# CHONSPQX/modulated-deform-conv

Hardware: AMD Instinct MI355X
Metric: fwd+bwd GSamples/s, MDCN2d 3x3 C=256 56x56 B=32; %HBM roofline (higher is better)
Workload: dtype f32; 1 GPU; ModulatedDeformConv2d 3x3, C_in=C_out=256, 56x56, deformable_group=1, fp32, B=32 per GPU, forward+backward (BASELINE.json configs[1]); global_batch=32, parallelism=dp1 batch-sharded

## Files before the change

### modulated_deform_conv_amd/csrc/mfma_fwd.hip

```cpp
#include "mfma_kernels.hpp"

#include <stdio.h>
#include <stdlib.h>
#include <string.h>

#include "mfma_tile.hpp"

namespace mdconv {

namespace {


template <int ND, bool MOD, int BM, int BN, int WM, int WN, bool PADK>
__global__ __launch_bounds__(256) void mfma_fwd_kernel(Geom g, PackDims pd,
                                                       const float *__restrict__ input,
                                                       const float *__restrict__ wp,
                                                       const float *__restrict__ bias,
                                                       const float *__restrict__ offset,
                                                       const float *__restrict__ mask,
                                                       float *__restrict__ output, int ntm, int ntn,
                                                       int full_tiles, int tail_ways, int tail_hi,
                                                       float *__restrict__ part) {
  constexpr int BK = kBK;
  constexpr int NC = 1 << ND;
  constexpr int NP = NC / 2;
  constexpr int MB = WM / 32, NB = WN / 32;
  constexpr int WAVES_N = BN / WN;
  constexpr int KSUBS = 256 / BN;
  constexpr int CPT = BK / KSUBS;
  static_assert((BM / WM) * (BN / WN) == 4, "4 waves per workgroup");
  static_assert(BK == 16 && CPT >= 1 && BN <= 256 && MB * 2 * 1024 <= 4096, "tile shape");

  __shared__ __attribute__((aligned(16))) float Bs[2 * BK * BN];

  const int grp = blockIdx.y;
  int tile, tap_lo = 0, tap_hi = g.K, tail_slot = -1;
  if ((int)blockIdx.x < full_tiles) {
    tile = xcd_remap(blockIdx.x, full_tiles);
  } else {
    tail_slot = blockIdx.x - full_tiles;
    const int hi_slots = tail_hi * (tail_ways + 1);
    int ti, way, wt;
    if (tail_slot < hi_slots) {
      wt = tail_ways + 1;
      ti = tail_slot / wt;
      way = tail_slot - ti * wt;
    } else {
      wt = tail_ways;
      const int r = tail_slot - hi_slots;
      ti = tail_hi + r / wt;
      way = r - (r / wt) * wt;
    }
    tile = full_tiles + ti;
    tap_lo = way * g.K / wt;
    tap_hi = (way + 1) * g.K / wt;
  }
  const int tn = tile / ntm, tm = tile - tn * ntm;
  const int o0 = tm * BM;
  const int n0 = tn * BN;

  const int tid = threadIdx.x;
  const int lane = tid & 63;
  const int wave = __builtin_amdgcn_readfirstlane(tid >> 6);
  const int wm0 = (wave / WAVES_N) * WM, wn0 = (wave % WAVES_N) * WN;
  const int kh = lane >> 5;

  const int j = tid % BN, ksub = tid / BN;
  const int n_g = min(n0 + j, g.N - 1);
  const int b_g = n_g / g.S_o;
  const int pix_g = n_g - b_g * g.S_o;
  int oc[ND];
  out_coords<ND>(g, pix_g, oc);

  const int cchunks = pd.Cgp / BK;
  const int T = g.K * cchunks;
  const int mblks = pd.Ogp / 32;
  const int slab_bytes = mblks * 2 * 64 * 4 * 4;

  const rsrc_t r_in = make_rsrc(input, (size_t)g.B * g.C * g.S_i * sizeof(float));
  const rsrc_t r_wp = make_rsrc(wp + (size_t)grp * T * (slab_bytes / 4), (size_t)T * slab_bytes);
  const int a_voff = (((o0 + wm0) / 32) * 2 * 64 + lane) * 16;
  const int img_voff = (b_g * g.C + grp * g.Cg + ksub * CPT) * g.S_i * 4;

  f32x16 acc[MB][NB];
#pragma unroll
  for (int i = 0; i < MB; ++i)
#pragma unroll
    for (int k = 0; k < NB; ++k)
#pragma unroll
      for (int r = 0; r < 16; ++r) acc[i][k][r] = 0.f;

  int voff[NP];
  float wgt[NC];
  float2 rg0[CPT][NP], rg1[CPT][NP];
  float wc0[NC], wc1[NC];
  int cur_tap = -1, cur_dg = -1;
  typedef unsigned long long lanemask_t;
  lanemask_t bad[NC], bad0[NC], bad1[NC];
#pragma unroll
  for (int ci = 0; ci < NC; ++ci) bad[ci] = bad0[ci] = bad1[ci] = 0ull;

  auto issue = [&](float2 (&rg)[CPT][NP], float (&wc)[NC], lanemask_t (&bd)[NC], int tap, int c0) {
    const int dg = g.DG == 1 ? 0 : min(grp * g.Cg + c0, g.C - 1) / g.Cdg;
    if (tap != cur_tap || dg != cur_dg) {
      float delta[ND];
      const int64_t ob = ((int64_t)(b_g * g.DG + dg) * (ND * g.K) + ND * tap) * g.S_o + pix_g;
#pragma unroll
      for (int a = 0; a < ND; ++a) delta[a] = offset[ob + (int64_t)a * g.S_o];
      int tcd[ND];
      tap_coords<ND>(g, tap, tcd);
      TapCoef<ND, float> tc;
      make_tap<ND, float>(g, oc, tcd, delta, false, tc);
      const float m = MOD ? mask[((int64_t)(b_g * g.DG + dg) * g.K + tap) * g.S_o + pix_g] : 1.f;
      int pidx[NP];
      float pwx[NP], pwy[NP];
      make_pairs<ND, float>(g, tc, m, pidx, pwx, pwy);
      bool prx[NP], pry[NP];
      make_pairs_read<ND, float>(g, tc, prx, pry);
#pragma unroll
      for (int pi = 0; pi < NP; ++pi) {
        voff[pi] = (prx[pi] || pry[pi]) ? img_voff + pidx[pi] * 4 : 0x7ffffff0;
        wgt[2 * pi] = pwx[pi];
        wgt[2 * pi + 1] = pwy[pi];
        bad[2 * pi] = __ballot(pry[pi] && !prx[pi]);
        bad[2 * pi + 1] = __ballot(prx[pi] && !pry[pi]);
      }
      cur_tap = tap;
      cur_dg = dg;
    }
    const int soff = c0 * g.S_i * 4;
#pragma unroll
    for (int i = 0; i < CPT; ++i)
#pragma unroll
      for (int pi = 0; pi < NP; ++pi) {
        rg[i][pi] = buf_load2(r_in, voff[pi], soff + i * g.S_i * 4);
      }
#pragma unroll
    for (int ci = 0; ci < NC; ++ci) { wc[ci] = wgt[ci]; bd[ci] = bad[ci]; }
  };
  auto commit = [&](const float2 (&rgl)[CPT][NP], const float (&wc)[NC], const lanemask_t (&bd)[NC], int c0, float *Bb) {
    lanemask_t any_bad = 0ull;
#pragma unroll
    for (int ci = 0; ci < NC; ++ci) any_bad |= bd[ci];
    float2 rg[CPT][NP];
#pragma unroll
    for (int i = 0; i < CPT; ++i)
#pragma unroll
      for (int pi = 0; pi < NP; ++pi) rg[i][pi] = rgl[i][pi];
    if (any_bad != 0ull) {
#pragma unroll
      for (int i = 0; i < CPT; ++i)
#pragma unroll
        for (int pi = 0; pi < NP; ++pi) {
          asm("v_cndmask_b32_e64 %0, %1, 0, %2" : "=v"(rg[i][pi].x) : "v"(rgl[i][pi].x), "s"(bd[2 * pi]));
          asm("v_cndmask_b32_e64 %0, %1, 0, %2" : "=v"(rg[i][pi].y) : "v"(rgl[i][pi].y), "s"(bd[2 * pi + 1]));
        }
    }
#pragma unroll
    for (int i = 0; i < CPT; ++i) {
      float val = wc[0] * rg[i][0].x;
      val = fmaf(wc[1], rg[i][0].y, val);
#pragma unroll
      for (int pi = 1; pi < NP; ++pi) {
        val = fmaf(wc[2 * pi], rg[i][pi].x, val);
        val = fmaf(wc[2 * pi + 1], rg[i][pi].y, val);
      }
      if (PADK) {
        const int cl = c0 + ksub * CPT + i;
        val = cl < g.Cg ? val : 0.f;
      }
      Bb[(ksub * CPT + i) * BN + j] = val;
    }
  };
  auto load_a = [&](float4 (&ra)[MB][2], int soff) {
#pragma unroll
    for (int i = 0; i < MB; ++i)
#pragma unroll
      for (int q = 0; q < 2; ++q) {
        ra[i][q] = buf_load4(r_wp, a_voff + (i * 2 + q) * 1024, soff);
      }
  };
  auto mma = [&](const float4 (&ra)[MB][2], const float *Bbuf) {
    const float *Bb = Bbuf + wn0 + (lane & 31) + 4 * kh * BN;
#pragma unroll
    for (int q = 0; q < 2; ++q)
#pragma unroll
      for (int s = 0; s < 4; ++s) {
        float b[NB];
#pragma unroll
        for (int n = 0; n < NB; ++n) b[n] = Bb[(8 * q + s) * BN + n * 32];
#pragma unroll
        for (int i = 0; i < MB; ++i) {
          const float a = s == 0 ? ra[i][q].x : (s == 1 ? ra[i][q].y : (s == 2 ? ra[i][q].z : ra[i][q].w));
#pragma unroll
          for (int n = 0; n < NB; ++n)
            acc[i][n] = __builtin_amdgcn_mfma_f32_32x32x2f32(a, b[n], acc[i][n], 0, 0, 0);
        }
      }
  };

  float4 ra0[MB][2], ra1[MB][2];
  const int a_last = (T - 1) * slab_bytes;
  int a_soff = tap_lo * cchunks * slab_bytes;
  load_a(ra0, a_soff);
  issue(rg0, wc0, bad0, tap_lo, 0);
  issue(rg1, wc1, bad1, tap_lo, BK);
  for (int tap = tap_lo; tap < tap_hi; ++tap) {
    for (int c0 = 0; c0 < pd.Cgp; c0 += 2 * BK) {
      const bool wrap = c0 + 2 * BK >= pd.Cgp;
      const int ntap = wrap ? min(tap + 1, g.K - 1) : tap;
      const int nc0 = wrap ? 0 : c0 + 2 * BK;
      commit(rg0, wc0, bad0, c0, Bs);
      __syncthreads();
      load_a(ra1, a_soff + slab_bytes);
      issue(rg0, wc0, bad0, ntap, nc0);
      __builtin_amdgcn_sched_barrier(0);
      mma(ra0, Bs);
      commit(rg1, wc1, bad1, c0 + BK, Bs + BK * BN);
      __syncthreads();
      a_soff += 2 * slab_bytes;
      load_a(ra0, min(a_soff, a_last));
      issue(rg1, wc1, bad1, ntap, nc0 + BK);
      __builtin_amdgcn_sched_barrier(0);
      mma(ra1, Bs + BK * BN);
    }
  }

  if (tail_slot >= 0) {
    float *dst = part + (size_t)tail_slot * (BM * BN) + wn0 + (lane & 31);
#pragma unroll
    for (int q = 0; q < NB; ++q)
#pragma unroll
      for (int mb = 0; mb < MB; ++mb)
#pragma unroll
        for (int r = 0; r < 16; ++r)
          dst[(wm0 + mb * 32 + (r & 3) + 8 * (r >> 2) + 4 * kh) * BN + q * 32] = acc[mb][q][r];
    return;
  }
#pragma unroll
  for (int q = 0; q < NB; ++q) {
    const int n_e = n0 + wn0 + q * 32 + (lane & 31);
    if (n_e < g.N) {
      const int b_e = n_e / g.S_o;
      const int pix_e = n_e - b_e * g.S_o;
#pragma unroll
      for (int mb = 0; mb < MB; ++mb)
#pragma unroll
        for (int r = 0; r < 16; ++r) {
          const int ol = o0 + wm0 + mb * 32 + (r & 3) + 8 * (r >> 2) + 4 * kh;
          if (ol < g.Og) {
            const int och = grp * g.Og + ol;
            const float bv = g.with_bias ? bias[och] : 0.f;
            output[(int64_t)(b_e * g.O + och) * g.S_o + pix_e] = acc[mb][q][r] + bv;
          }
        }
    }
  }
}

constexpr int kTailSlices = 16;
template <int BM, int BN>
__global__ __launch_bounds__(256) void fwd_tail_reduce_kernel(Geom g, const float *__restrict__ part,
                                                              const float *__restrict__ bias,
                                                              float *__restrict__ output, int ntm,
                                                              int full_tiles, int tail_ways, int tail_hi) {
  const int tile = full_tiles + blockIdx.x;
  const int tn = tile / ntm, tm = tile - tn * ntm;
  const int ti = blockIdx.x;
  const int slot0 = ti < tail_hi ? ti * (tail_ways + 1) : tail_hi * (tail_ways + 1) + (ti - tail_hi) * tail_ways;
  const int nways = ti < tail_hi ? tail_ways + 1 : tail_ways;
  const float *src = part + (size_t)slot0 * (BM * BN);
  const int e_lo = blockIdx.y * (BM * BN / kTailSlices);
  for (int e = e_lo + threadIdx.x; e < e_lo + BM * BN / kTailSlices; e += 256) {
    const int ol = tm * BM + e / BN, n = tn * BN + e % BN;
    if (ol >= g.Og || n >= g.N) continue;
    float sacc = src[e];
    for (int w = 1; w < nways; ++w) sacc += src[(size_t)w * (BM * BN) + e];
    const int b = n / g.S_o, pix = n - b * g.S_o;
    output[(int64_t)(b * g.O + ol) * g.S_o + pix] = sacc + (g.with_bias ? bias[ol] : 0.f);
  }
}

}

void fwd_tail_plan(const Geom &g, int tiles, int slots, int *full_tiles, int *ways, int *n_hi) {
  static const int tail_env = getenv("MDCONV_FWD_TAIL") ? atoi(getenv("MDCONV_FWD_TAIL")) : 2;
  *full_tiles = tiles;
  *ways = 1;
  *n_hi = 0;
  if (!tail_env || g.G != 1 || g.K < 2 || slots <= 0) return;
  const int rem = tiles % slots;
  if (rem == 0) return;
  int w = slots / rem;
  const int cap = g.K < 4 ? g.K : 4;
  if (tail_env == 1) {
    if (tiles < slots) return;
    if (w > cap) w = cap;
    if (w < 2) return;
    *full_tiles = tiles - rem;
    *ways = w;
    return;
  }
  if (w >= cap) {
    *full_tiles = tiles - rem;
    *ways = cap;
    return;
  }
  const int hi = slots - rem * w;
  if (w == 1) {
    if (hi == 0) return;
    *full_tiles = tiles - hi;
    *ways = 1;
    *n_hi = hi;
    return;
  }
  *full_tiles = tiles - rem;
  *ways = w;
  *n_hi = hi;
}

int fwd_tail_reduce_launch(int BM, int BN, const Geom &g, const float *part, const float *bias, float *output, int ntm,
                           int tail_tiles, int full_tiles, int ways, int n_hi, hipStream_t stream) {
  if (tail_tiles <= 0) return MDCONV_OK;
#define FWD_TAIL_RED(M, N)                                                                                        \
  hipLaunchKernelGGL((fwd_tail_reduce_kernel<M, N>), dim3(tail_tiles, kTailSlices), dim3(256), 0, stream, g, part, bias, \
                     output, ntm, full_tiles, ways, n_hi)
  if (BM == 256 && BN == 32) FWD_TAIL_RED(256, 32);
  else if (BM == 128 && BN == 64) FWD_TAIL_RED(128, 64);
  else if (BM == 64 && BN == 128) FWD_TAIL_RED(64, 128);
  else if (BM == 64 && BN == 64) FWD_TAIL_RED(64, 64);
  else { set_error("fwd_tail_reduce: no instance for a %d x %d tile", BM, BN); return MDCONV_ELAUNCH; }
#undef FWD_TAIL_RED
  return check_launch("fwd_tail_reduce");
}

namespace {
template <int ND, bool MOD, int BM, int BN, int WM, int WN, bool PADK>
int fwd_tile_slots() {
  static int slots = 0;
  if (!slots) {
    int n = 0;
    (void)hipOccupancyMaxActiveBlocksPerMultiprocessor(
        &n, reinterpret_cast<const void *>(&mfma_fwd_kernel<ND, MOD, BM, BN, WM, WN, PADK>), 256, 0);
    (void)hipGetLastError();
    slots = device_cus() * (n > 0 ? (n < kTailMaxPerCu ? n : kTailMaxPerCu) : 3);
  }
  return slots;
}

template <int ND, bool MOD, int BM, int BN, int WM, int WN, bool PADK>
int launch_fwd_tile_k(const Geom &g, const PackDims &pd, const Tensors &t, const float *wp, float *part,
                      hipStream_t stream) {
  const int ntm = (g.Og + BM - 1) / BM;
  const int ntn = (g.N + BN - 1) / BN;
  int full_tiles, ways, n_hi;
  fwd_tail_plan(g, ntm * ntn, part ? fwd_tile_slots<ND, MOD, BM, BN, WM, WN, PADK>() : 0, &full_tiles, &ways, &n_hi);
  const int tail_tiles = ntm * ntn - full_tiles;
  static const bool debug_plan = getenv("MDCONV_DEBUG_PLAN") != nullptr;
  if (debug_plan)
    fprintf(stderr, "[mdconv] forward plan: %d x %d tile, %d tiles, slots %d, full %d, tail %d x %d tap ranges (%d of them x %d)\n", BM, BN,
            ntm * ntn, part ? fwd_tile_slots<ND, MOD, BM, BN, WM, WN, PADK>() : 0, full_tiles, tail_tiles, ways, n_hi, ways + 1);
  dim3 grid(full_tiles + tail_tiles * ways + n_hi, g.G);
  hipLaunchKernelGGL((mfma_fwd_kernel<ND, MOD, BM, BN, WM, WN, PADK>), grid, dim3(256), 0, stream,
                     g, pd, (const float *)t.input, wp, (const float *)t.bias,
                     (const float *)t.offset, (const float *)t.mask, (float *)t.output, ntm, ntn,
                     full_tiles, ways, n_hi, part);
  int rc = check_launch("mfma_fwd");
  if (rc || tail_tiles == 0) return rc;
  return fwd_tail_reduce_launch(BM, BN, g, part, (const float *)t.bias, (float *)t.output, ntm, tail_tiles, full_tiles, ways,
                                n_hi, stream);
}

template <int ND, bool MOD, int BM, int BN, int WM, int WN>
int launch_fwd_tile(const Geom &g, const PackDims &pd, const Tensors &t, const float *wp, float *part,
                    hipStream_t stream) {
  if (g.Cg % (2 * kBK)) return launch_fwd_tile_k<ND, MOD, BM, BN, WM, WN, true>(g, pd, t, wp, part, stream);
  return launch_fwd_tile_k<ND, MOD, BM, BN, WM, WN, false>(g, pd, t, wp, part, stream);
}

template <int ND, bool MOD>
int launch_fwd(const Geom &g, const PackDims &pd, const Tensors &t, const float *wp, float *part,
               hipStream_t stream) {
  if (pd.BM == 256) return launch_fwd_tile<ND, MOD, 256, 32, 64, 32>(g, pd, t, wp, part, stream);
  if (pd.BM == 128) return launch_fwd_tile<ND, MOD, 128, 64, 64, 32>(g, pd, t, wp, part, stream);
  return launch_fwd_tile<ND, MOD, 64, 128, 64, 32>(g, pd, t, wp, part, stream);
}

}


size_t fwd_tail_bytes(const Geom &g) {
  return g.G == 1 && g.K >= 2 ? (size_t)device_cus() * kTailMaxPerCu * 8192 * sizeof(float) : 0;
}

int mfma_forward_f32(const Geom &g, const PackDims &pd, const Tensors &t, const float *wp, float *part,
                     hipStream_t stream) {
  if (g.nd == 2)
    return g.modulated ? launch_fwd<2, true>(g, pd, t, wp, part, stream)
                       : launch_fwd<2, false>(g, pd, t, wp, part, stream);
  return g.modulated ? launch_fwd<3, true>(g, pd, t, wp, part, stream)
                     : launch_fwd<3, false>(g, pd, t, wp, part, stream);
}

}
```

Baseline: 70.78 GSamples/s.

## Precompute per-tap bilinear sampling state into an LDS table in forward kernel

Adds a templated variant of the forward MFMA kernel that, in a prologue, has the threads of a workgroup split the taps between them, computing offsets, mask, bilinear weights, voffsets and boundary flags once per tap and pixel into a dynamic LDS table. The main loop then fetches each tap's state from LDS at the tap boundary instead of recomputing it from global offset and mask loads inside issue. The table is enabled only when deformable_group is 1, it fits in 64 KiB, and occupancy does not drop. The cost is extra LDS use, a prologue barrier, and a restructured tap-wrap loop.

Result: no change. 71.12 GSamples/s (median of 6 runs) (+0.5%).

```diff
diff --git a/modulated_deform_conv_amd/csrc/mfma_fwd.hip b/modulated_deform_conv_amd/csrc/mfma_fwd.hip
--- a/modulated_deform_conv_amd/csrc/mfma_fwd.hip
+++ b/modulated_deform_conv_amd/csrc/mfma_fwd.hip
@@ -1,5 +1,7 @@
 #include "mfma_kernels.hpp"
 
+#include <map>
+#include <mutex>
 #include <stdio.h>
 #include <stdlib.h>
 #include <string.h>
@@ -11,7 +13,9 @@
 namespace {
 
 
-template <int ND, bool MOD, int BM, int BN, int WM, int WN, bool PADK>
+template <int ND> constexpr int fwd_row_dwords() { return ND == 2 ? 8 : 16; }
+
+template <int ND, bool MOD, int BM, int BN, int WM, int WN, bool PADK, bool TBL>
 __global__ __launch_bounds__(256) void mfma_fwd_kernel(Geom g, PackDims pd,
                                                        const float *__restrict__ input,
                                                        const float *__restrict__ wp,
@@ -32,6 +36,8 @@
   static_assert(BK == 16 && CPT >= 1 && BN <= 256 && MB * 2 * 1024 <= 4096, "tile shape");
 
   __shared__ __attribute__((aligned(16))) float Bs[2 * BK * BN];
+  extern __shared__ __attribute__((aligned(16))) int Tb[];
+  constexpr int ROWD = fwd_row_dwords<ND>();
 
   const int grp = blockIdx.y;
   int tile, tap_lo = 0, tap_hi = g.K, tail_slot = -1;
@@ -80,7 +86,9 @@
   const rsrc_t r_in = make_rsrc(input, (size_t)g.B * g.C * g.S_i * sizeof(float));
   const rsrc_t r_wp = make_rsrc(wp + (size_t)grp * T * (slab_bytes / 4), (size_t)T * slab_bytes);
   const int a_voff = (((o0 + wm0) / 32) * 2 * 64 + lane) * 16;
-  const int img_voff = (b_g * g.C + grp * g.Cg + ksub * CPT) * g.S_i * 4;
+  const int img_base = (b_g * g.C + grp * g.Cg) * g.S_i * 4;
+  const int ksub_voff = ksub * CPT * g.S_i * 4;
+  constexpr int kParked = 0x7ffffff0;
 
   f32x16 acc[MB][NB];
 #pragma unroll
@@ -100,33 +108,93 @@
 #pragma unroll
   for (int ci = 0; ci < NC; ++ci) bad[ci] = bad0[ci] = bad1[ci] = 0ull;
 
+  auto make_state = [&](int tap, int dg, int base, int (&vo)[NP], float (&w)[NC], bool (&bx)[NP], bool (&by)[NP]) {
+    float delta[ND];
+    const int64_t ob = ((int64_t)(b_g * g.DG + dg) * (ND * g.K) + ND * tap) * g.S_o + pix_g;
+#pragma unroll
+    for (int a = 0; a < ND; ++a) delta[a] = offset[ob + (int64_t)a * g.S_o];
+    int tcd[ND];
+    tap_coords<ND>(g, tap, tcd);
+    TapCoef<ND, float> tc;
+    make_tap<ND, float>(g, oc, tcd, delta, false, tc);
+    const float m = MOD ? mask[((int64_t)(b_g * g.DG + dg) * g.K + tap) * g.S_o + pix_g] : 1.f;
+    int pidx[NP];
+    float pwx[NP], pwy[NP];
+    make_pairs<ND, float>(g, tc, m, pidx, pwx, pwy);
+    bool prx[NP], pry[NP];
+    make_pairs_read<ND, float>(g, tc, prx, pry);
+#pragma unroll
+    for (int pi = 0; pi < NP; ++pi) {
+      vo[pi] = (prx[pi] || pry[pi]) ? base + pidx[pi] * 4 : kParked;
+      w[2 * pi] = pwx[pi];
+      w[2 * pi + 1] = pwy[pi];
+      bx[pi] = pry[pi] && !prx[pi];
+      by[pi] = prx[pi] && !pry[pi];
+    }
+  };
+  if (TBL) {
+#pragma unroll 1
+    for (int tap = tap_lo + ksub; tap < tap_hi; tap += KSUBS) {
+      int vo[NP];
+      float w[NC];
+      bool bx[NP], by[NP];
+      make_state(tap, 0, img_base, vo, w, bx, by);
+      int row[ROWD];
+      int flags = 0;
+#pragma unroll
+      for (int pi = 0; pi < NP; ++pi) {
+        row[pi] = vo[pi];
+        flags |= (bx[pi] ? 1 << (2 * pi) : 0) | (by[pi] ? 2 << (2 * pi) : 0);
+      }
+#pragma unroll
+      for (int ci = 0; ci < NC; ++ci) row[NP + ci] = __float_as_int(w[ci]);
+      row[NP + NC] = flags;
+#pragma unroll
+      for (int i = NP + NC + 1; i < ROWD; ++i) row[i] = 0;
+      int *dst = Tb + ((tap - tap_lo) * BN + j) * ROWD;
+#pragma unroll
+      for (int i = 0; i < ROWD; i += 4) *reinterpret_cast<int4 *>(dst + i) = make_int4(row[i], row[i + 1], row[i + 2], row[i + 3]);
+    }
+    __syncthreads();
+  }
+
+  auto fetch_state = [&](int tap) {
+    const int *src = Tb + (min(tap, tap_hi - 1) - tap_lo) * (BN * ROWD) + j * ROWD;
+    int row[ROWD];
+#pragma unroll
+    for (int i = 0; i < ROWD; i += 4) {
+      const int4 q = *reinterpret_cast<const int4 *>(src + i);
+      row[i] = q.x; row[i + 1] = q.y; row[i + 2] = q.z; row[i + 3] = q.w;
+    }
+#pragma unroll
+    for (int pi = 0; pi < NP; ++pi)
+      voff[pi] = max(row[pi], (int)((unsigned)row[pi] + (unsigned)ksub_voff));
+#pragma unroll
+    for (int ci = 0; ci < NC; ++ci) wgt[ci] = __int_as_float(row[NP + ci]);
+    const int flags = row[NP + NC];
+    if (__ballot(flags != 0) != 0ull) {
+#pragma unroll
+      for (int ci = 0; ci < NC; ++ci) bad[ci] = __ballot((flags >> ci) & 1);
+    } else {
+#pragma unroll
+      for (int ci = 0; ci < NC; ++ci) bad[ci] = 0ull;
+    }
+  };
+
   auto issue = [&](float2 (&rg)[CPT][NP], float (&wc)[NC], lanemask_t (&bd)[NC], int tap, int c0) {
-    const int dg = g.DG == 1 ? 0 : min(grp * g.Cg + c0, g.C - 1) / g.Cdg;
-    if (tap != cur_tap || dg != cur_dg) {
-      float delta[ND];
-      const int64_t ob = ((int64_t)(b_g * g.DG + dg) * (ND * g.K) + ND * tap) * g.S_o + pix_g;
-#pragma unroll
-      for (int a = 0; a < ND; ++a) delta[a] = offset[ob + (int64_t)a * g.S_o];
-      int tcd[ND];
-      tap_coords<ND>(g, tap, tcd);
-      TapCoef<ND, float> tc;
-      make_tap<ND, float>(g, oc, tcd, delta, false, tc);
-      const float m = MOD ? mask[((int64_t)(b_g * g.DG + dg) * g.K + tap) * g.S_o + pix_g] : 1.f;
-      int pidx[NP];
-      float pwx[NP], pwy[NP];
-      make_pairs<ND, float>(g, tc, m, pidx, pwx, pwy);
-      bool prx[NP], pry[NP];
-      make_pairs_read<ND, float>(g, tc, prx, pry);
-#pragma unroll
-      for (int pi = 0; pi < NP; ++pi) {
-        voff[pi] = (prx[pi] || pry[pi]) ? img_voff + pidx[pi] * 4 : 0x7ffffff0;
-        wgt[2 * pi] = pwx[pi];
-        wgt[2 * pi + 1] = pwy[pi];
-        bad[2 * pi] = __ballot(pry[pi] && !prx[pi]);
-        bad[2 * pi + 1] = __ballot(prx[pi] && !pry[pi]);
-      }
-      cur_tap = tap;
-      cur_dg = dg;
+    if (!TBL) {
+      const int dg = g.DG == 1 ? 0 : min(grp * g.Cg + c0, g.C - 1) / g.Cdg;
+      if (tap != cur_tap || dg != cur_dg) {
+        bool bx[NP], by[NP];
+        make_state(tap, dg, img_base + ksub_voff, voff, wgt, bx, by);
+#pragma unroll
+        for (int pi = 0; pi < NP; ++pi) {
+          bad[2 * pi] = __ballot(bx[pi]);
+          bad[2 * pi + 1] = __ballot(by[pi]);
+        }
+        cur_tap = tap;
+        cur_dg = dg;
+      }
     }
     const int soff = c0 * g.S_i * 4;
 #pragma unroll
@@ -203,26 +271,35 @@
   const int a_last = (T - 1) * slab_bytes;
   int a_soff = tap_lo * cchunks * slab_bytes;
   load_a(ra0, a_soff);
+  if (TBL) fetch_state(tap_lo);
   issue(rg0, wc0, bad0, tap_lo, 0);
   issue(rg1, wc1, bad1, tap_lo, BK);
+  auto chunk_pair = [&](int c0, int ntap, int nc0) {
+    commit(rg0, wc0, bad0, c0, Bs);
+    __syncthreads();
+    load_a(ra1, a_soff + slab_bytes);
+    issue(rg0, wc0, bad0, ntap, nc0);
+    __builtin_amdgcn_sched_barrier(0);
+    mma(ra0, Bs);
+    commit(rg1, wc1, bad1, c0 + BK, Bs + BK * BN);
+    __syncthreads();
+    a_soff += 2 * slab_bytes;
+    load_a(ra0, min(a_soff, a_last));
+    issue(rg1, wc1, bad1, ntap, nc0 + BK);
+    __builtin_amdgcn_sched_barrier(0);
+    mma(ra1, Bs + BK * BN);
+  };
   for (int tap = tap_lo; tap < tap_hi; ++tap) {
-    for (int c0 = 0; c0 < pd.Cgp; c0 += 2 * BK) {
-      const bool wrap = c0 + 2 * BK >= pd.Cgp;
-      const int ntap = wrap ? min(tap + 1, g.K - 1) : tap;
-      const int nc0 = wrap ? 0 : c0 + 2 * BK;
-      commit(rg0, wc0, bad0, c0, Bs);
-      __syncthreads();
-      load_a(ra1, a_soff + slab_bytes);
-      issue(rg0, wc0, bad0, ntap, nc0);
-      __builtin_amdgcn_sched_barrier(0);
-      mma(ra0, Bs);
-      commit(rg1, wc1, bad1, c0 + BK, Bs + BK * BN);
-      __syncthreads();
-      a_soff += 2 * slab_bytes;
-      load_a(ra0, min(a_soff, a_last));
-      issue(rg1, wc1, bad1, ntap, nc0 + BK);
-      __builtin_amdgcn_sched_barrier(0);
-      mma(ra1, Bs + BK * BN);
+    if (TBL) {
+      for (int c0 = 0; c0 + 2 * BK < pd.Cgp; c0 += 2 * BK) chunk_pair(c0, tap, c0 + 2 * BK);
+      const int ntap = min(tap + 1, g.K - 1);
+      fetch_state(ntap);
+      chunk_pair(pd.Cgp - 2 * BK, ntap, 0);
+    } else {
+      for (int c0 = 0; c0 < pd.Cgp; c0 += 2 * BK) {
+        const bool wrap = c0 + 2 * BK >= pd.Cgp;
+        chunk_pair(c0, wrap ? min(tap + 1, g.K - 1) : tap, wrap ? 0 : c0 + 2 * BK);
+      }
     }
   }
 
@@ -335,17 +412,28 @@
 }
 
 namespace {
+template <int ND, bool MOD, int BM, int BN, int WM, int WN, bool PADK, bool TBL>
+int fwd_tile_occupancy(size_t dyn) {
+  static std::mutex mu;
+  static std::map<size_t, int> cache;
+  std::lock_guard<std::mutex> lock(mu);
+  auto it = cache.find(dyn);
+  if (it != cache.end()) return it->second;
+  int n = 0;
+  (void)hipOccupancyMaxActiveBlocksPerMultiprocessor(
+      &n, reinterpret_cast<const void *>(&mfma_fwd_kernel<ND, MOD, BM, BN, WM, WN, PADK, TBL>), 256, dyn);
+  (void)hipGetLastError();
+  cache[dyn] = n;
+  return n;
+}
+
 template <int ND, bool MOD, int BM, int BN, int WM, int WN, bool PADK>
-int fwd_tile_slots() {
-  static int slots = 0;
-  if (!slots) {
-    int n = 0;
-    (void)hipOccupancyMaxActiveBlocksPerMultiprocessor(
-        &n, reinterpret_cast<const void *>(&mfma_fwd_kernel<ND, MOD, BM, BN, WM, WN, PADK>), 256, 0);
-    (void)hipGetLastError();
-    slots = device_cus() * (n > 0 ? (n < kTailMaxPerCu ? n : kTailMaxPerCu) : 3);
-  }
-  return slots;
+size_t fwd_table_bytes(const Geom &g) {
+  if (g.DG != 1) return 0;
+  const size_t bytes = (size_t)g.K * BN * fwd_row_dwords<ND>() * 4;
+  if (bytes + 2 * kBK * BN * 4 > 64 * 1024) return 0;
+  const int plain = fwd_tile_occupancy<ND, MOD, BM, BN, WM, WN, PADK, false>(0);
+  return fwd_tile_occupancy<ND, MOD, BM, BN, WM, WN, PADK, true>(bytes) >= plain && plain > 0 ? bytes : 0;
 }
 
 template <int ND, bool MOD, int BM, int BN, int WM, int WN, bool PADK>
@@ -353,18 +441,31 @@
                       hipStream_t stream) {
   const int ntm = (g.Og + BM - 1) / BM;
   const int ntn = (g.N + BN - 1) / BN;
+  const size_t tbl = fwd_table_bytes<ND, MOD, BM, BN, WM, WN, PADK>(g);
+  int slots = 0;
+  if (part) {
+    const int n = tbl ? fwd_tile_occupancy<ND, MOD, BM, BN, WM, WN, PADK, true>(tbl)
+                      : fwd_tile_occupancy<ND, MOD, BM, BN, WM, WN, PADK, false>(0);
+    slots = device_cus() * (n > 0 ? (n < kTailMaxPerCu ? n : kTailMaxPerCu) : 3);
+  }
   int full_tiles, ways, n_hi;
-  fwd_tail_plan(g, ntm * ntn, part ? fwd_tile_slots<ND, MOD, BM, BN, WM, WN, PADK>() : 0, &full_tiles, &ways, &n_hi);
+  fwd_tail_plan(g, ntm * ntn, slots, &full_tiles, &ways, &n_hi);
   const int tail_tiles = ntm * ntn - full_tiles;
   static const bool debug_plan = getenv("MDCONV_DEBUG_PLAN") != nullptr;
   if (debug_plan)
-    fprintf(stderr, "[mdconv] forward plan: %d x %d tile, %d tiles, slots %d, full %d, tail %d x %d tap ranges (%d of them x %d)\n", BM, BN,
-            ntm * ntn, part ? fwd_tile_slots<ND, MOD, BM, BN, WM, WN, PADK>() : 0, full_tiles, tail_tiles, ways, n_hi, ways + 1);
+    fprintf(stderr, "[mdconv] forward plan: %d x %d tile, %d tiles, slots %d, full %d, tail %d x %d tap ranges (%d of them x %d), state table %d bytes\n", BM, BN,
+            ntm * ntn, slots, full_tiles, tail_tiles, ways, n_hi, ways + 1, (int)tbl);
   dim3 grid(full_tiles + tail_tiles * ways + n_hi, g.G);
-  hipLaunchKernelGGL((mfma_fwd_kernel<ND, MOD, BM, BN, WM, WN, PADK>), grid, dim3(256), 0, stream,
-                     g, pd, (const float *)t.input, wp, (const float *)t.bias,
-                     (const float *)t.offset, (const float *)t.mask, (float *)t.output, ntm, ntn,
-                     full_tiles, ways, n_hi, part);
+  if (tbl)
+    hipLaunchKernelGGL((mfma_fwd_kernel<ND, MOD, BM, BN, WM, WN, PADK, true>), grid, dim3(256), tbl, stream,
+                       g, pd, (const float *)t.input, wp, (const float *)t.bias,
+                       (const float *)t.offset, (const float *)t.mask, (float *)t.output, ntm, ntn,
+                       full_tiles, ways, n_hi, part);
+  else
+    hipLaunchKernelGGL((mfma_fwd_kernel<ND, MOD, BM, BN, WM, WN, PADK, false>), grid, dim3(256), 0, stream,
+                       g, pd, (const float *)t.input, wp, (const float *)t.bias,
+                       (const float *)t.offset, (const float *)t.mask, (float *)t.output, ntm, ntn,
+                       full_tiles, ways, n_hi, part);
   int rc = check_launch("mfma_fwd");
   if (rc || tail_tiles == 0) return rc;
   return fwd_tail_reduce_launch(BM, BN, g, part, (const float *)t.bias, (float *)t.output, ntm, tail_tiles, full_tiles, ways,
```
